# chenruduan/OAReactDiff

Hardware: AMD Instinct MI355X
Metric: denoising_steps_per_sec (higher is better)
Workload: dtype f32; 1 GPU; EGNNDynamics.forward (LEFTNet H=196 R=96 L=6), B=64 reactions/GPU x 3 objects x 23 atoms, complete graph per reaction (N=4416, E=300288), T=1000 sampler step shape; batch_per_gpu=64, atoms_per_object=23, parallelism=replica x1 (no collective), launch=eager

## Files before the change

### oareactdiff_amd/_capi.py

```python
from __future__ import annotations

import ctypes as C
import os

from .build import LIB

OARD_MAX_OBJECTS = 8
ABI_VERSION = 2040
OARD_OK, OARD_EINVAL, OARD_ENOTCOMPLETE, OARD_EHIP, OARD_ENOMEM = 0, -1, -2, -3, -4
ERRORS = {OARD_EINVAL: "invalid argument / unsupported configuration", OARD_ENOTCOMPLETE: "topology is not complete-per-sample",
          OARD_EHIP: "HIP runtime error", OARD_ENOMEM: "workspace too small"}

PREC_GCL_BF16X3, PREC_EQUI_BF16X3, PREC_TRAIN_BF16X3 = 1, 2, 4
TAP_S, TAP_VEC, TAP_EDGE, TAP_POS_FRAME, TAP_DPOS, TAP_HOUT, TAP_LABELS, TAP_NE1 = 1, 2, 3, 4, 5, 6, 7, 8

EXPORTS = ["oard_version", "oard_supported", "oard_param_count", "oard_packed_bytes", "oard_pack_weights",
           "oard_topology_create", "oard_topology_destroy", "oard_topology_num_nodes", "oard_topology_num_edges",
           "oard_topology_num_inner_edges", "oard_topology_num_samples", "oard_topology_check_edge_index",
           "oard_workspace_bytes", "oard_forward", "oard_active_inner_edges", "oard_debug_lin3u_table", "oard_sampler_step", "oard_sampler_step_dev", "oard_tap", "oard_debug_stop_after", "oard_debug_option", "oard_timing_enable", "oard_timing_reset",
           "oard_timing_get",
           "oard_topology_create_parts", "oard_topology_export", "oard_tape_bytes", "oard_tape_entry", "oard_forward_train",
           "oard_packed_bwd_bytes", "oard_pack_weights_bwd", "oard_gcl_backward_dx", "oard_edge_node_sums",
           "oard_equi_backward_dx", "oard_scalarize_backward", "oard_equi_msg_backward", "oard_lin3u_forward", "oard_lin3u_backward", "oard_wgrad_scratch_bytes", "oard_wgrad",
           "oard_train_scratch_bytes", "oard_train_scratch_poison", "oard_train_scratch_entry", "oard_train_tail_backward",
# ... 114 lines not shown
    L.oard_library_stream.argtypes = [ci, pvp]; L.oard_library_stream.restype = ci
    L.oard_graph_create.argtypes = [cfgp, vp, vp, i64, vp, i64, pvp]; L.oard_graph_create.restype = ci
    L.oard_graph_destroy.argtypes = [vp]; L.oard_graph_destroy.restype = None
    L.oard_graph_num_nodes.argtypes = [vp]; L.oard_graph_num_nodes.restype = i64
    L.oard_graph_num_edges.argtypes = [vp]; L.oard_graph_num_edges.restype = i64
    L.oard_graph_object_rows.argtypes = [vp, ci]; L.oard_graph_object_rows.restype = i64
    L.oard_graph_is_complete.argtypes = [vp]; L.oard_graph_is_complete.restype = ci
    L.oard_graph_workspace_bytes.argtypes = [cfgp, vp]; L.oard_graph_workspace_bytes.restype = sz
    L.oard_graph_forward.argtypes = [cfgp, vp, pvp, sz, pvp, vp, ci, vp, pvp, vp, sz, vp, vp]; L.oard_graph_forward.restype = ci
    L.oard_debug_stop_after.argtypes = [C.c_int]; L.oard_debug_stop_after.restype = C.c_int
    L.oard_debug_option.argtypes = [C.c_char_p, C.c_int]; L.oard_debug_option.restype = C.c_int
    L.oard_timing_enable.argtypes = [C.c_int]; L.oard_timing_enable.restype = C.c_int
    L.oard_timing_reset.argtypes = []; L.oard_timing_reset.restype = C.c_int
    L.oard_timing_get.argtypes = [C.c_char_p, C.POINTER(C.c_double), C.POINTER(i64)]; L.oard_timing_get.restype = C.c_int
    for env, opt in (("OARD_GCL_VARIANT", b"gcl_variant"), ("OARD_EQUI_VARIANT", b"equi_variant"),
                     ("OARD_NODE_VARIANT", b"node_variant"), ("OARD_GCL_SKIP", b"gcl_skip"), ("OARD_EQUI_SKIP", b"equi_skip"), ("OARD_EQUI_L0_SKIP", b"equi_l0_skip"), ("OARD_GCL_MSUM", b"gcl_msum"), ("OARD_GCL_PERSIST", b"gcl_persist"), ("OARD_GCL_GRID", b"gcl_grid"), ("OARD_PARTS", b"parts"), ("OARD_SEQUENTIAL", b"sequential"), ("OARD_POISON", b"poison"), ("OARD_AUTO_SMALL", b"auto_small"), ("OARD_AUTO_TINY", b"auto_tiny"), ("OARD_NPB", b"npb"),
                     ("OARD_WGRAD_WGS", b"wgrad_wgs"), ("OARD_WGRAD_LDS", b"wgrad_lds"), ("OARD_WGRAD_T16", b"wgrad_t16"), ("OARD_WGRAD_QUEUE", b"wgrad_queue"), ("OARD_GATE_FOLD", b"gate_fold"), ("OARD_WGRAD_SHAPES", b"wgrad_shapes"), ("OARD_TRAIN_DUAL", b"train_dual"), ("OARD_SMALL_SPLIT", b"small_split"),
                     ("OARD_SKIP_FAMILIES", b"skip_families")):
        if os.environ.get(env) not in (None, ""):
            check(L.oard_debug_option(opt, int(os.environ[env])), f"oard_debug_option({opt.decode()})")
    _lib = L
    return L


def timing_get(family: str):
    ms, n = C.c_double(0.0), C.c_int64(0)
    check(lib().oard_timing_get(family.encode(), C.byref(ms), C.byref(n)), "oard_timing_get")
    return ms.value, n.value
```

### oareactdiff_amd/csrc/oard_hip.hip

```cpp
#include <algorithm>
#include <cmath>
#include <cstdio>
#include <cstring>
#include <map>
#include <string>
#include <vector>
#include <mutex>
#include <chrono>
#include <utility>

#include "oard_kernels.h"
#include "oard_edge_v1.h"
#include "oard_edge_p.h"
#include "oard_wgrad_t16.h"
#include "oard_edge_b3.h"
#ifdef OARD_EXPERIMENTS
#include "oard_edge_fp.h"
#endif
#include "oard_node_v1.h"
#include "oard_edge_small.h"
#include "oard_edge_bwd.h"
#include "oard_node_bwd.h"
#include "oard_rows.h"
#include "oard_inst.h"
// ... 33 lines not shown
        }
        recs.clear();
    }
} g_timing;
int g_stop_after = 0;
int g_gcl_variant = 2;
int g_equi_variant = 2;
int g_sequential = 0;
int g_auto_tiny = 8;
int g_auto_small = 4;
int g_npb = 0;
int g_poison = 0;
int g_equi_l0_skip = 1;
int g_gcl_msum = 1;
int g_gcl_msum_taken = 0;
int g_equi_l0_taken = 0;
int g_parts = 0;
int g_small_split = 128;
int g_wgrad_shapes = 3;
int g_wgrad_t16 = 256;
int g_wgrad_lds = 256;
int g_wgrad_wgs = 512;
int g_gcl_persist = 1;
int g_gcl_grid = 0;
int g_equi_skip = 1;
int g_gcl_skip = 1;
int g_node_variant = 1;
int g_skip_families = 0;

struct ScopedLaunch {
// ... 517 lines not shown
    } else if constexpr (kV0) {
        LAUNCH(F_INIT, (k_neighbor<D>), gN, 256, st, tp, wb, po, (const float*)zemb, (const float*)nb, (const float*)ew, s_at(0), s1);
        LAUNCH(F_INIT, (k_s2v_agg<D>), gN, 256, st, tp, (const float*)s1, (const float*)ew, (const float*)geo, ne1);
    } else return OARD_EINVAL;
    if (A > 0) LAUNCH2(F_INIT, (k_scalarize<D>), gA, (gA * topo->conc <= 2048 ? D::HT : 1), 256, st, tp, wb, po, (const float*)ne1, (const float*)geo, ew);
    HIP_TRY(hipMemsetAsync(vec, 0, (size_t)N * 3 * D::HP * sizeof(float), st));
    if (stop_after == 1) return OARD_OK;

    float* vec2 = (float*)(ws + w.vec2);
    float* vcur = vec;
    float* vnext = vec2;
    const bool msum = !train && g_gcl_msum && E > 0 && gcl_variant == 2 && node_variant == 1 && equi_variant != 0 && tp.npb > 4 &&
                      (tp.CI == 0 || gcl_v1_throughput(c->precision, gcl_variant, topo->conc, tp.CI)) &&
                      (tp.CX == 0 || gcl_v1_throughput(c->precision, gcl_variant, topo->conc, tp.CX));
    g_gcl_msum_taken = msum;
    for (int l = 0; l < c->num_layers; ++l) {
        const LayerOff lo = po.layer[l];
        const bool nv1 = node_variant == 1 && equi_variant != 0;
        const unsigned gN16 = (unsigned)cdiv(N, tp.npb);
        float* ew_in = ew_at(l);
        float* ew_out = ew_at(l + 1);
        if (train) vnext = (float*)(tape + to.vec_in[l + 1]);

        if (nv1) LAUNCH(F_NODE, (k_node_pre_v1<D, NW>), gN16, NW * 64, st, tp, wb, po, lo, (const float*)s_at(l), (const float*)pp0, xhb, P, Q);
        else if constexpr (kV0) LAUNCH(F_NODE, (k_node_pre<D>), gN, 256, st, tp, wb, po, lo, (const float*)s, (const float*)pp0, xhb, P, Q);
        else return OARD_EINVAL;
        if (E > 0) {
            if (gcl_variant == 0) {
                if constexpr (kV0) LAUNCH(F_GCL_EDGE, (k_gcl_edge<D>), gE, 256, st, tp, wb, lo, (const float*)P, (const float*)Q, ew_in, mbuf);
                else return OARD_EINVAL;
// ... 23 lines not shown
                       s, vcur, v2buf, scal, vdot);
            } else return OARD_EINVAL;
        } else {
            const bool l0_skip = l == 0 && !train && g_equi_l0_skip && A > 0 && nv1 && !rows &&
                                 equi_v1_shape(c->precision, equi_variant, topo->conc, A, (const float*)(ws + w.d1s)) == 2;
            if (l == 0) g_equi_l0_taken = l0_skip;
            if (A > 0) {
                int rc = launch_equi_v1<D>(c->precision, equi_variant, topo->conc, tp, wb, lo, wb + lo.equi_stream, wb + lo.dp0b, ew_out, rbuf, vmsg,
                                           train ? (float*)(tape + to.zd1[l]) : nullptr, train ? (float*)(tape + to.cd[l]) : nullptr, st,
                                           (float*)(ws + w.d1s), al, l0_skip);
                if (rc != OARD_OK) return rc;
            }
#define EQUI_NODE_V1(D_, ROWS_, XC_) LAUNCH(F_NODE, (k_equi_node_v1<D_, NW, ROWS_, XC_>), gN16, NW * 64, st, tp, wb, lo, (const float*)vmsg, \
                       (const float*)xq, (const float*)geo, (const float*)x1, (const float*)s_mid_at(l), s_at(l + 1), (const float*)vcur, vnext, \
                       train ? (float*)(tape + to.s_a[l]) : nullptr, train ? (float*)(tape + to.vec_a[l]) : nullptr, al)
            if (nv1 && rows) {
                if (lo.xcross) EQUI_NODE_V1(D, true, true); else EQUI_NODE_V1(D, true, false);
            } else if (nv1 && l0_skip) {
                if (lo.xcross) EQUI_NODE_V1(Layer0<D>, false, true); else EQUI_NODE_V1(Layer0<D>, false, false);
            } else if (nv1) {
                if (lo.xcross) EQUI_NODE_V1(D, false, true); else EQUI_NODE_V1(D, false, false);
            } else if constexpr (kV0) {
                LAUNCH(F_NODE, (k_equi_agg_v1<D>), gN, 256, st, tp, wb, lo, (const float*)vmsg, (const float*)xq,
                       (const float*)geo, (const float*)x1, s, (const float*)vcur, vnext, v2buf, scal, vdot);
            } else return OARD_EINVAL;
            std::swap(vcur, vnext);
        }
        if constexpr (kV0) {
            if (!nv1) LAUNCH(F_NODE, (k_equi_upd<D>), gN, 256, st, tp, wb, lo, (const float*)scal, (const float*)vdot,
                             (const float*)v2buf, s, vcur);
        }
        if (stop_after == 100 + 10 * l + 2) { topo->vec_final = (size_t)((char*)vcur - ws); return OARD_OK; }
// ... 1535 lines not shown
    return OARD_OK;
}

int oard_debug_stop_after(int code) { g_stop_after = code; return OARD_OK; }
int oard_debug_option(const char* name, int value) {
    if (!name) return OARD_EINVAL;
    if (!kV0 && value == 0 && (strcmp(name, "gcl_variant") == 0 || strcmp(name, "equi_variant") == 0 || strcmp(name, "node_variant") == 0))
        return OARD_EINVAL;
    if (strcmp(name, "gcl_variant") == 0) { g_gcl_variant = value; return OARD_OK; }
    if (strcmp(name, "equi_variant") == 0) { g_equi_variant = value; return OARD_OK; }
    if (strcmp(name, "node_variant") == 0) { g_node_variant = value; return OARD_OK; }
    if (strcmp(name, "experiments") == 0) return kV0 ? OARD_OK : OARD_EINVAL;
    if (strcmp(name, "gcl_skip") == 0) { g_gcl_skip = value; return OARD_OK; }
    if (strcmp(name, "equi_skip") == 0) { g_equi_skip = value; return OARD_OK; }
    if (strcmp(name, "equi_l0_skip") == 0) { g_equi_l0_skip = value; return OARD_OK; }
    if (strcmp(name, "gcl_msum") == 0) { g_gcl_msum = value; return OARD_OK; }
    if (strcmp(name, "gcl_msum_taken") == 0) return g_gcl_msum_taken ? OARD_OK : OARD_EINVAL;
    if (strcmp(name, "equi_l0_taken") == 0) return g_equi_l0_taken ? OARD_OK : OARD_EINVAL;
    if (strcmp(name, "gcl_persist") == 0) { g_gcl_persist = value; return OARD_OK; }
    if (strcmp(name, "gcl_grid") == 0) { g_gcl_grid = value; return OARD_OK; }
    if (strcmp(name, "skip_families") == 0) { g_skip_families = value; return OARD_OK; }
    if (strcmp(name, "parts") == 0) { g_parts = value; return OARD_OK; }
    if (strcmp(name, "sequential") == 0) { g_sequential = value; return OARD_OK; }
    if (strcmp(name, "poison") == 0) { g_poison = value; return OARD_OK; }
    if (strcmp(name, "auto_small") == 0) { g_auto_small = value; return OARD_OK; }
    if (strcmp(name, "auto_tiny") == 0) { g_auto_tiny = value; return OARD_OK; }
    if (strcmp(name, "npb") == 0) { g_npb = value; return OARD_OK; }
    if (strcmp(name, "wgrad_wgs") == 0) { g_wgrad_wgs = value; return OARD_OK; }
    if (strcmp(name, "wgrad_t16") == 0) { g_wgrad_t16 = value; return OARD_OK; }
    if (strcmp(name, "wgrad_queue") == 0) { g_wgrad_queue = value; return OARD_OK; }
// ... 49 lines not shown
```

### oareactdiff_amd/csrc/oard_inst.h

```cpp
#pragma once
#if !defined(OARD_EXPERIMENTS) && !defined(OARD_SINGLE_TU)

#define OARD_UNPAREN(...) __VA_ARGS__
#ifdef OARD_INST_DEFINE
#define OARD_INST(K, ARGS) template __global__ void OARD_UNPAREN K ARGS;
#else
#define OARD_INST(K, ARGS) extern template __global__ void OARD_UNPAREN K ARGS;
#endif
#ifndef OARD_DIMS_LIST
#define OARD_DIMS_LIST X(196, 96) X(32, 8) X(32, 32)
#endif
#define OARD_BOOL4(M, D) M(D, true, true) M(D, false, true) M(D, true, false) M(D, false, false)

#define OARD_NW(h) (((h) + 15) / 16 <= 16 ? ((h) + 15) / 16 : 8)
#define OARD_A_GCL (TopoDev, const float*, const float*, const float*, const float*, const float*, long long, long long, const float*, float*, float*, GclTape)

#if !defined(OARD_INST_DEFINE) || defined(OARD_INST_UNIT_GCL_P)
#define OARD_I_GCL_P(D, S1, S3) OARD_INST((k_gcl_edge_p<OARD_UNPAREN D, S1, S3, false>), OARD_A_GCL) OARD_INST((k_gcl_edge_p<OARD_UNPAREN D, S1, S3, true>), OARD_A_GCL) \
    OARD_INST((k_gcl_edge_p<OARD_UNPAREN D, S1, S3, false, true>), OARD_A_GCL)
#define X(h, r) OARD_BOOL4(OARD_I_GCL_P, (Dims<h, r>))
OARD_DIMS_LIST
#undef X
#endif

// ... 24 lines not shown
    OARD_INST((k_equi_edge_v1<Dims<h, r>, 4, false>), OARD_A_EQUI) \
    OARD_INST((k_equi_node_v1<Dims<h, r>, OARD_NW(h), false, false>), OARD_A_EQUI_NODE) OARD_INST((k_equi_node_v1<Dims<h, r>, OARD_NW(h), false, true>), OARD_A_EQUI_NODE) \
    OARD_INST((k_equi_node_v1<Dims<h, r>, OARD_NW(h), true, false>), OARD_A_EQUI_NODE) OARD_INST((k_equi_node_v1<Dims<h, r>, OARD_NW(h), true, true>), OARD_A_EQUI_NODE) \
    OARD_INST((k_equi_node_v1<Layer0<Dims<h, r> >, OARD_NW(h), false, false>), OARD_A_EQUI_NODE) OARD_INST((k_equi_node_v1<Layer0<Dims<h, r> >, OARD_NW(h), false, true>), OARD_A_EQUI_NODE) \
    OARD_INST((k_gcl_edge_bwd<Dims<h, r>, 8, 2, true>), (TopoDev, const float*, long long, long long, GclBwdArgs)) \
    OARD_INST((k_gcl_edge_bwd<Dims<h, r>, 8, 2, false>), (TopoDev, const float*, long long, long long, GclBwdArgs)) \
    OARD_INST((k_equi_edge_bwd<Dims<h, r>, 8>), (TopoDev, const float*, const float*, const float*, float*, float*))
OARD_DIMS_LIST
#undef X
#endif

#if !defined(OARD_INST_DEFINE) || defined(OARD_INST_UNIT_NODE)
#define OARD_A_GCL_NODE (TopoDev, const float*, LayerOff, const float*, const float*, float*, float*, float*)
#define OARD_A_OUT (TopoDev, const float*, PackOff, const float*, const float*, float*, float*, int*)
#define OARD_A_SCAL_BWD (TopoDev, const float*, const float*, int, const float*, const float*, float*, float*)
#define OARD_A_MSG_BWD (TopoDev, const float*, Strided3, Strided3, const float*, Strided3, const float*, int, Strided3, float*, float*, float*, float*, int, int, int)
#define X(h, r) \
    OARD_INST((k_gcl_node_v1<Dims<h, r>, OARD_NW(h), false>), OARD_A_GCL_NODE) OARD_INST((k_gcl_node_v1<Dims<h, r>, OARD_NW(h), true>), OARD_A_GCL_NODE) \
    OARD_INST((k_gcl_node_v1<Dims<h, r>, OARD_NW(h), false, true>), OARD_A_GCL_NODE) \
    OARD_INST((k_out_v1<Dims<h, r>, OARD_NW(h)>), OARD_A_OUT) \
    OARD_INST((k_scalarize_bwd<Dims<h, r>, 2, false>), OARD_A_SCAL_BWD) OARD_INST((k_scalarize_bwd<Dims<h, r>, 2, true>), OARD_A_SCAL_BWD) \
    OARD_INST((k_equi_msg_bwd<Dims<h, r> >), OARD_A_MSG_BWD)
OARD_DIMS_LIST
#undef X
OARD_INST((k_lin3u_bwd_fused<4>), (const float*, const float*, const float*, long long, float*, float*))
#define OARD_I_ROWS(KB, EPI) OARD_INST((k_rows_dense<KB, EPI, 8>), (RowsDense)) OARD_INST((k_rows_dense_long<KB, EPI, 8, 4>), (RowsDense))
OARD_I_ROWS(13, 0) OARD_I_ROWS(13, 2) OARD_I_ROWS(13, 3) OARD_I_ROWS(7, 3) OARD_I_ROWS(6, 0) OARD_I_ROWS(6, 1) OARD_I_ROWS(4, 1) OARD_I_ROWS(4, 3)
OARD_INST((k_rows_dense<26, 1, 8>), (RowsDense)) OARD_INST((k_rows_dense<26, 3, 8>), (RowsDense))
OARD_INST((k_rows_dense2<13, 1, 8, 13>), (RowsDense2)) OARD_INST((k_rows_dense2<13, 2, 8, 13>), (RowsDense2))
OARD_INST((k_rows_dense2<26, 1, 8, 13>), (RowsDense2)) OARD_INST((k_rows_dense2<39, 2, 8, 13>), (RowsDense2))
#endif

#if !defined(OARD_INST_DEFINE) || defined(OARD_INST_UNIT_WGRAD)
#define OARD_A_WG (const float*, int, int, const float*, int, int, long long, long long, long long, int, int, float*, float*, float*)
OARD_INST((k_wgrad_t16<4, 7, false>), (WgtArgs)) OARD_INST((k_wgrad_t16<4, 7, true>), (WgtArgs)) OARD_INST((k_wgrad_t16<5, 3, false>), (WgtArgs))
OARD_INST((k_wgrad_t16<5, 5, true>), (WgtArgs)) OARD_INST((k_wgrad_t16<5, 7, true>), (WgtArgs)) OARD_INST((k_wgrad_t16<6, 5, false>), (WgtArgs))
OARD_INST((k_wgrad_t16<6, 7, false>), (WgtArgs))
// ... 7 lines not shown
```

### oareactdiff_amd/csrc/oard_node_v1.h

```cpp
#pragma once
#include "oard_kernels.h"

OARD_DEV f4 lds_blk(const float* v, int b, int lane) { return *reinterpret_cast<const f4*>(v + b * 256 + lane * 4); }
OARD_DEV void lds_st(float* v, int t, int lane, f4 x) { *reinterpret_cast<f4*>(v + t * 256 + lane * 4) = x; }

#ifndef OARD_NODE_PF
#define OARD_NODE_PF 13
#endif
template <int KB>
OARD_DEV f4 dense_tile_lds(const float* __restrict__ wp, int t, const float* in, int lane, f4 init) {
    const float* base = wp + ((size_t)t * KB * 64 + lane) * 4;
    f4 c0 = init, c1 = f4zero();
    constexpr int G = OARD_NODE_PF;
#pragma unroll
    for (int b0 = 0; b0 < KB; b0 += G) {
        f4 a[G];
#pragma unroll
        for (int i = 0; i < G; ++i)
            if (b0 + i < KB) a[i] = ld_f4(base + (size_t)(b0 + i) * 256);
        __builtin_amdgcn_sched_barrier(0);
#pragma unroll
        for (int i = 0; i < G; ++i)
            if (b0 + i < KB) {
                const f4 x = lds_blk(in, b0 + i, lane);
// ... 431 lines not shown
#pragma unroll
    for (int j = 0; j < 8; ++j) h2[j] = b2[j];
#pragma unroll 4
    for (int k = 0; k < 48; ++k) {
        const f4 wa = *reinterpret_cast<const f4*>(l3s + 12 * k), wc = *reinterpret_cast<const f4*>(l3s + 12 * k + 4);
        const float h = silu1(x * l3s[12 * k + 8] + l3s[12 * k + 9]);
        h2[0] += h * wa.x; h2[1] += h * wa.y; h2[2] += h * wa.z; h2[3] += h * wa.w;
        h2[4] += h * wc.x; h2[5] += h * wc.y; h2[6] += h * wc.z; h2[7] += h * wc.w;
    }
    float o = p[592];
#pragma unroll
    for (int j = 0; j < 8; ++j) o += silu1(h2[j]) * w4[j];
    return o;
}

template <class D> struct Layer0 : D {};
template <class D> struct is_layer0 { static constexpr bool value = false; };
template <class D> struct is_layer0<Layer0<D> > { static constexpr bool value = true; };
template <class D, int WAVES, bool ROWS = false, bool XC = false>
__global__ __launch_bounds__(WAVES * 64) void k_equi_node_v1(TopoDev tp, const float* __restrict__ wb, LayerOff lo,
                                                             const float* __restrict__ qbuf, const float* __restrict__ xq,
                                                             const float* __restrict__ geo, const float* __restrict__ x1,
                                                             const float* s, float* s_out, const float* __restrict__ vec_in,
                                                             float* __restrict__ vec_out,
                                                             float* __restrict__ sa_out, float* __restrict__ va_out ,
                                                             ActList al ) {
    constexpr bool L0 = is_layer0<D>::value;
    static_assert(!(L0 && ROWS), "the layer-0 form exists for the large-batch gather only");
    constexpr int HT = D::HT;
    constexpr int TPW = (HT + WAVES - 1) / WAVES;
    __shared__ __attribute__((aligned(16))) float sm[6 * HT * 256 + 48 * 12 + L3T_FLOATS];
    float* l3s = sm + 6 * HT * 256;
    float* l3t = l3s + 48 * 12;
#ifdef OARD_NO_L3T
    const bool l3t_ok = false;
#else
    const bool l3t_ok = tp.npb > 4 && (wb + lo.l3t)[2 * (L3T_N + 1)] > 0.5f;
#endif
    if (l3t_ok)
        for (int i = threadIdx.x; i < 2 * (L3T_N + 1) / 4; i += WAVES * 64)
            reinterpret_cast<f4*>(l3t)[i] = ld_f4(wb + lo.l3t + 4 * i);
    if (l3t_ok && threadIdx.x < 2) l3t[2 * (L3T_N + 1) - 2 + threadIdx.x] = (wb + lo.l3t)[2 * (L3T_N + 1) - 2 + threadIdx.x];
#ifdef OARD_TIMELINE
    const bool tl_on_ = blockIdx.x == gridDim.x / 2 && (threadIdx.x & 63) == 0; int tl_n_ = 0;
#endif
    TL(1);
    lin3u_stage(wb + lo.l3u, l3s, threadIdx.x, WAVES * 64);
    float* vx = sm;
    float* in = sm + 3 * HT * 256;
    float* hx = sm + 5 * HT * 256;
    const NodeBlk nb = node_blk(tp.N, tp.npb);
    const int n = nb.n;
    const bool listed = al.pre != nullptr && (long long)__builtin_amdgcn_readfirstlane(*al.n) != tp.A;
    const int a0 = listed ? al.pre[tp.act_ptr[n]] : tp.act_ptr[n];
    const int cnt = nb.valid ? (listed ? al.pre[tp.act_ptr[n + 1]] : tp.act_ptr[n + 1]) - a0 : 0;
    const int mx = wave_max(cnt);
    auto row_of = [&](int k) -> int { return listed ? al.rows[k] : k; };
// ... 16 lines not shown
                     zn2 = ld_blk(xq, nn, 3 * D::HP, 2 * HT + t, nb.lane);
            for (int k = 0; k < mx2; k += rl.L) {
                const int kk = k + rl.slot;
                const int ke = min(b0 + min(kk, max(cnt2 - 1, 0)), a_hi);
                const size_t a = cnt2 > 0 ? (size_t)row_of(ke) : 0;
                const int m = cnt2 > 0 ? src_of(ke) : 0;
                const float* gp = geo + a * GEO_STRIDE;
                const float gx = gp[2], gy = gp[3], gz = gp[4];
                const float cx = XC ? gp[5] : 0.f, cy = XC ? gp[6] : 0.f, cz = XC ? gp[7] : 0.f;
                const f4 q0 = ld_blk(qbuf, a, 3 * D::HP, t, nb.lane), q1 = ld_blk(qbuf, a, 3 * D::HP, HT + t, nb.lane),
                         q2 = ld_blk(qbuf, a, 3 * D::HP, 2 * HT + t, nb.lane);
                const f4 y0 = ld_blk(xq, m, 3 * D::HP, t, nb.lane), y1 = ld_blk(xq, m, 3 * D::HP, HT + t, nb.lane),
                         y2 = ld_blk(xq, m, 3 * D::HP, 2 * HT + t, nb.lane);
                const f4 w0 = ld_blk(vec_in, (size_t)m * 3 + 0, D::HP, t, nb.lane), w1 = ld_blk(vec_in, (size_t)m * 3 + 1, D::HP, t, nb.lane),
                         w2 = ld_blk(vec_in, (size_t)m * 3 + 2, D::HP, t, nb.lane);
                if (kk < cnt2) {
                    const f4 xm = (y0 + zn0) * q0;
                    dx += xm;
                    const f4 a2 = (y1 + zn1) * q1 * inv_sqrt3;
                    const f4 a3 = (y2 + zn2) * q2;
                    v0 += (XC ? w0 * a2 + a3 * gx + xm * cx : w0 * a2 + a3 * gx) * inv_sqrt_h;
                    v1 += (XC ? w1 * a2 + a3 * gy + xm * cy : w1 * a2 + a3 * gy) * inv_sqrt_h;
                    v2 += (XC ? w2 * a2 + a3 * gz + xm * cz : w2 * a2 + a3 * gz) * inv_sqrt_h;
                }
            }
            dx = rows_total4(dx, rl, nb.lane); v0 = rows_total4(v0, rl, nb.lane);
            v1 = rows_total4(v1, rl, nb.lane); v2 = rows_total4(v2, rl, nb.lane);
        }
        int mnext[2], rnext[2];
        auto entry = [&](int kk, int& m, int& r) {
            const int ke = min(a0 + min(kk, max(cnt - 1, 0)), a_hi);
            m = cnt > 0 ? src_of(ke) : 0;
            r = cnt > 0 ? row_of(ke) : 0;
        };
#pragma unroll
        for (int i = 0; i < 2; ++i) entry(i, mnext[i], rnext[i]);
        float zero1 = 0.f;
        if (L0) asm volatile("" : "+v"(zero1));
        const f4 zero4 = {zero1, zero1, zero1, zero1};
// ... 9 lines not shown
                const size_t a = (size_t)rc[i];
                const int m = mc[i];
                const float* g = geo + a * GEO_STRIDE;
                gx[i] = g[2]; gy[i] = g[3]; gz[i] = g[4];
                cx[i] = XC ? g[5] : 0.f; cy[i] = XC ? g[6] : 0.f; cz[i] = XC ? g[7] : 0.f;
                q0[i] = ld_blk(qbuf, a, 3 * D::HP, t, nb.lane); q1[i] = L0 ? zero4 : ld_blk(qbuf, a, 3 * D::HP, HT + t, nb.lane);
                q2[i] = ld_blk(qbuf, a, 3 * D::HP, 2 * HT + t, nb.lane);
                y0[i] = ld_blk(xq, m, 3 * D::HP, t, nb.lane); y1[i] = L0 ? zero4 : ld_blk(xq, m, 3 * D::HP, HT + t, nb.lane);
                y2[i] = ld_blk(xq, m, 3 * D::HP, 2 * HT + t, nb.lane);
                w0[i] = L0 ? zero4 : ld_blk(vec_in, (size_t)m * 3 + 0, D::HP, t, nb.lane);
                w1[i] = L0 ? zero4 : ld_blk(vec_in, (size_t)m * 3 + 1, D::HP, t, nb.lane);
                w2[i] = L0 ? zero4 : ld_blk(vec_in, (size_t)m * 3 + 2, D::HP, t, nb.lane);
            }
#pragma unroll
            for (int i = 0; i < 2; ++i)
                if (k + i < cnt) {
                    const f4 xm = (y0[i] + xn0) * q0[i];
                    dx += xm;
                    const f4 a2 = (y1[i] + xn1) * q1[i] * inv_sqrt3;
                    const f4 a3 = (y2[i] + xn2) * q2[i];
                    v0 += (XC ? w0[i] * a2 + a3 * gx[i] + xm * cx[i] : w0[i] * a2 + a3 * gx[i]) * inv_sqrt_h;
                    v1 += (XC ? w1[i] * a2 + a3 * gy[i] + xm * cy[i] : w1[i] * a2 + a3 * gy[i]) * inv_sqrt_h;
                    v2 += (XC ? w2[i] * a2 + a3 * gz[i] + xm * cz[i] : w2[i] * a2 + a3 * gz[i]) * inv_sqrt_h;
                }
        }
        const f4 sa = (ld_blk(s, n, D::HP, t, nb.lane) + dx) * inv_sqrt2;
        v0 += ld_blk(vec_in, (size_t)n * 3 + 0, D::HP, t, nb.lane);
        v1 += ld_blk(vec_in, (size_t)n * 3 + 1, D::HP, t, nb.lane);
        v2 += ld_blk(vec_in, (size_t)n * 3 + 2, D::HP, t, nb.lane);
        lds_st(in, t, nb.lane, sa);
        lds_st(vx + 0 * HT * 256, t, nb.lane, v0);
        lds_st(vx + 1 * HT * 256, t, nb.lane, v1);
        lds_st(vx + 2 * HT * 256, t, nb.lane, v2);
        if (sa_out != nullptr && nb.valid) {
            st_blk(sa_out, n, D::HP, t, nb.lane, sa);
            st_blk(va_out, (size_t)n * 3 + 0, D::HP, t, nb.lane, v0);
            st_blk(va_out, (size_t)n * 3 + 1, D::HP, t, nb.lane, v1);
            st_blk(va_out, (size_t)n * 3 + 2, D::HP, t, nb.lane, v2);
        }
    }
    TL(2);
    __syncthreads();
    TL(3);

    const float fx = x1[n * 3], fy = x1[n * 3 + 1], fz = x1[n * 3 + 2];
    const float* l3 = wb + lo.l3u;
    f4 v2k[TPW][3], vdk[TPW];
#pragma unroll
    for (int i = 0; i < TPW; ++i) {
        const int t = nb.wave + i * WAVES;
        if (t < HT) {
            TileJob job[2] = {tile_job<HT>(wb + lo.vp, t, vx), tile_job<HT>(wb + lo.vp, HT + t, vx)};
            f4 acc[6];
#pragma unroll
            for (int k = 0; k < 6; ++k) acc[k] = f4zero();
            dense_seq_xyz<HT, 2, HT * 256, (ROWS ? 5 : OARD_NODE_SEQ_G), ROWS>(job, nb.lane, acc);
            const f4 v1[3] = {acc[0], acc[1], acc[2]}, v2[3] = {acc[3], acc[4], acc[5]};
#pragma unroll
            for (int x = 0; x < 3; ++x) v2k[i][x] = v2[x];
            const f4 sc = v1[0] * fx + v1[1] * fy + v1[2] * fz;
            vdk[i] = (v1[0] * v2[0] + v1[1] * v2[1] + v1[2] * v2[2]) * inv_sqrt_h;
            f4 sca;
            const int f0 = 16 * t + 4 * nb.g;
            if (tp.npb <= 4) {
                float* blk = in + (HT + t) * 256;
                lds_st(in, HT + t, nb.lane, sc);
                __builtin_amdgcn_wave_barrier();
                const int f = nb.lane >> 2, c = nb.lane & 3;
                float* cell = blk + (16 * (f >> 2) + c) * 4 + (f & 3);
                const float y = (c < tp.npb && 16 * t + f < D::H) ? lin3u1(l3s, l3, *cell) : 0.f;
                *cell = y;
            } else {
                const bool in_tab = fabsf(sc.x) < L3T_X && fabsf(sc.y) < L3T_X && fabsf(sc.z) < L3T_X && fabsf(sc.w) < L3T_X;
                if (l3t_ok && !__any(!in_tab))
                    sca = (f4){lin3u_table_eval(l3t, sc.x), lin3u_table_eval(l3t, sc.y), lin3u_table_eval(l3t, sc.z), lin3u_table_eval(l3t, sc.w)};
                else
                    sca = lin3u4(l3s, l3, sc);
                sca.x = f0 + 0 < D::H ? sca.x : 0.f; sca.y = f0 + 1 < D::H ? sca.y : 0.f;
                sca.z = f0 + 2 < D::H ? sca.z : 0.f; sca.w = f0 + 3 < D::H ? sca.w : 0.f;
                lds_st(in, HT + t, nb.lane, sca);
            }
        }
    }
    TL(4);
    __syncthreads();
    TL(5);

    {
        TileJob job[TPW];
        f4 acc[TPW];
#pragma unroll
        for (int i = 0; i < TPW; ++i) { job[i] = tile_job<2 * HT>(wb + lo.xv0, min(nb.wave + i * WAVES, HT - 1), in); acc[i] = f4zero(); }
        dense_seq<2 * HT, TPW>(job, nb.lane, acc);
#pragma unroll
        for (int i = 0; i < TPW; ++i)
            if (nb.wave + i * WAVES < HT) lds_st(hx, nb.wave + i * WAVES, nb.lane, silu4(acc[i]));
    }
    TL(6);
    __syncthreads();
    TL(7);

    {
        TileJob job[3 * TPW];
        f4 acc[3 * TPW];
#pragma unroll
        for (int i = 0; i < TPW; ++i) {
            const int t = min(nb.wave + i * WAVES, HT - 1);
#pragma unroll
            for (int k = 0; k < 3; ++k) { job[3 * i + k] = tile_job<HT>(wb + lo.xv2, k * HT + t, hx); acc[3 * i + k] = f4zero(); }
        }
        dense_seq<HT, 3 * TPW>(job, nb.lane, acc);
#pragma unroll
        for (int i = 0; i < TPW; ++i) {
            const int t = nb.wave + i * WAVES;
            if (t < HT && nb.valid) {
                const f4 a = acc[3 * i], b = acc[3 * i + 1], c = acc[3 * i + 2];
                st_blk(s_out, n, D::HP, t, nb.lane, lds_blk(in, t, nb.lane) + (a + b + vdk[i]) * inv_sqrt2);
#pragma unroll
                for (int x = 0; x < 3; ++x)
                    st_blk(vec_out, (size_t)n * 3 + x, D::HP, t, nb.lane,
                           lds_blk(vx + x * HT * 256, t, nb.lane) + c * v2k[i][x]);
            }
        }
    }
    TL(0);
    TL_END();
}

template <class D, int WAVES>
__global__ __launch_bounds__(WAVES * 64) void k_neighbor_v1(TopoDev tp, const float* __restrict__ wb, PackOff po,
                                                            const float* __restrict__ zemb, const float* __restrict__ nbe,
                                                            const float* __restrict__ ew, float* __restrict__ s,
                                                            float* __restrict__ s1) {
    constexpr int HT = D::HT, TPW = (HT + WAVES - 1) / WAVES;
    __shared__ __attribute__((aligned(16))) float sm[2 * HT * 256];
    float* sv = sm;
    float* yv = sm + HT * 256;
    const NodeBlk nb = node_blk(tp.N, tp.npb);
    const int n = nb.n, smp = tp.node_sample[n], s0 = tp.sample_ptr[smp];
    const int ns = nb.valid ? tp.sample_ptr[smp + 1] - s0 : 0;
    const int mx = wave_max(ns);
// ... 210 lines not shown
```

Baseline: 3698 reaction-steps/s.

## Split equivariant node kernel into per-feature gather and dense update kernels

Adds an inference-only path that breaks the fused equivariant node kernel in two. A wave-per-64-features gather kernel accumulates edge messages directly from global memory into s and a vector buffer. A separate block-tiled update kernel then reloads those into LDS and runs the dense projections. The gather is meant to get better parallelism and latency hiding than the LDS-heavy fused kernel, at the cost of an extra kernel launch and a global round trip for the intermediate s/vec. The shared math is factored into helpers, and message accumulation now uses explicit FMAs with contraction disabled.

```diff
diff --git a/oareactdiff_amd/_capi.py b/oareactdiff_amd/_capi.py
--- a/oareactdiff_amd/_capi.py
+++ b/oareactdiff_amd/_capi.py
@@ -152,7 +152,7 @@
     L.oard_timing_reset.argtypes = []; L.oard_timing_reset.restype = C.c_int
     L.oard_timing_get.argtypes = [C.c_char_p, C.POINTER(C.c_double), C.POINTER(i64)]; L.oard_timing_get.restype = C.c_int
     for env, opt in (("OARD_GCL_VARIANT", b"gcl_variant"), ("OARD_EQUI_VARIANT", b"equi_variant"),
-                     ("OARD_NODE_VARIANT", b"node_variant"), ("OARD_GCL_SKIP", b"gcl_skip"), ("OARD_EQUI_SKIP", b"equi_skip"), ("OARD_EQUI_L0_SKIP", b"equi_l0_skip"), ("OARD_GCL_MSUM", b"gcl_msum"), ("OARD_GCL_PERSIST", b"gcl_persist"), ("OARD_GCL_GRID", b"gcl_grid"), ("OARD_PARTS", b"parts"), ("OARD_SEQUENTIAL", b"sequential"), ("OARD_POISON", b"poison"), ("OARD_AUTO_SMALL", b"auto_small"), ("OARD_AUTO_TINY", b"auto_tiny"), ("OARD_NPB", b"npb"),
+                     ("OARD_NODE_VARIANT", b"node_variant"), ("OARD_GCL_SKIP", b"gcl_skip"), ("OARD_EQUI_SKIP", b"equi_skip"), ("OARD_EQUI_L0_SKIP", b"equi_l0_skip"), ("OARD_EQUI_SPLIT", b"equi_split"), ("OARD_GCL_MSUM", b"gcl_msum"), ("OARD_GCL_PERSIST", b"gcl_persist"), ("OARD_GCL_GRID", b"gcl_grid"), ("OARD_PARTS", b"parts"), ("OARD_SEQUENTIAL", b"sequential"), ("OARD_POISON", b"poison"), ("OARD_AUTO_SMALL", b"auto_small"), ("OARD_AUTO_TINY", b"auto_tiny"), ("OARD_NPB", b"npb"),
                      ("OARD_WGRAD_WGS", b"wgrad_wgs"), ("OARD_WGRAD_LDS", b"wgrad_lds"), ("OARD_WGRAD_T16", b"wgrad_t16"), ("OARD_WGRAD_QUEUE", b"wgrad_queue"), ("OARD_GATE_FOLD", b"gate_fold"), ("OARD_WGRAD_SHAPES", b"wgrad_shapes"), ("OARD_TRAIN_DUAL", b"train_dual"), ("OARD_SMALL_SPLIT", b"small_split"),
                      ("OARD_SKIP_FAMILIES", b"skip_families")):
         if os.environ.get(env) not in (None, ""):
diff --git a/oareactdiff_amd/csrc/oard_hip.hip b/oareactdiff_amd/csrc/oard_hip.hip
--- a/oareactdiff_amd/csrc/oard_hip.hip
+++ b/oareactdiff_amd/csrc/oard_hip.hip
@@ -71,6 +71,8 @@
 int g_equi_l0_skip = 1;
 int g_gcl_msum = 1;
 int g_gcl_msum_taken = 0;
+int g_equi_split = 1;
+int g_equi_split_taken = 0;
 int g_equi_l0_taken = 0;
 int g_parts = 0;
 int g_small_split = 128;
@@ -618,6 +620,8 @@
                       (tp.CI == 0 || gcl_v1_throughput(c->precision, gcl_variant, topo->conc, tp.CI)) &&
                       (tp.CX == 0 || gcl_v1_throughput(c->precision, gcl_variant, topo->conc, tp.CX));
     g_gcl_msum_taken = msum;
+    const bool equi_split = !train && g_equi_split && A > 0 && node_variant == 1 && equi_variant != 0 && tp.npb > 4;
+    g_equi_split_taken = equi_split;
     for (int l = 0; l < c->num_layers; ++l) {
         const LayerOff lo = po.layer[l];
         const bool nv1 = node_variant == 1 && equi_variant != 0;
@@ -671,8 +675,14 @@
 #define EQUI_NODE_V1(D_, ROWS_, XC_) LAUNCH(F_NODE, (k_equi_node_v1<D_, NW, ROWS_, XC_>), gN16, NW * 64, st, tp, wb, lo, (const float*)vmsg, \
                        (const float*)xq, (const float*)geo, (const float*)x1, (const float*)s_mid_at(l), s_at(l + 1), (const float*)vcur, vnext, \
                        train ? (float*)(tape + to.s_a[l]) : nullptr, train ? (float*)(tape + to.vec_a[l]) : nullptr, al)
+#define EQUI_GATHER_V1(D_, XC_) LAUNCH(F_NODE, (k_equi_gather_v1<D_, XC_>), (unsigned)cdiv(N * ((D::HP + 63) / 64), 4), 256, st, tp, (const float*)vmsg, \
+                       (const float*)xq, (const float*)geo, s, (const float*)vcur, vnext, al)
             if (nv1 && rows) {
                 if (lo.xcross) EQUI_NODE_V1(D, true, true); else EQUI_NODE_V1(D, true, false);
+            } else if (nv1 && equi_split) {
+                if (l0_skip) { if (lo.xcross) EQUI_GATHER_V1(Layer0<D>, true); else EQUI_GATHER_V1(Layer0<D>, false); }
+                else { if (lo.xcross) EQUI_GATHER_V1(D, true); else EQUI_GATHER_V1(D, false); }
+                LAUNCH(F_NODE, (k_equi_update_v1<D, NW>), gN16, NW * 64, st, tp, wb, lo, (const float*)x1, s, vnext);
             } else if (nv1 && l0_skip) {
                 if (lo.xcross) EQUI_NODE_V1(Layer0<D>, false, true); else EQUI_NODE_V1(Layer0<D>, false, false);
             } else if (nv1) {
@@ -2238,6 +2248,8 @@
     if (strcmp(name, "gcl_skip") == 0) { g_gcl_skip = value; return OARD_OK; }
     if (strcmp(name, "equi_skip") == 0) { g_equi_skip = value; return OARD_OK; }
     if (strcmp(name, "equi_l0_skip") == 0) { g_equi_l0_skip = value; return OARD_OK; }
+    if (strcmp(name, "equi_split") == 0) { g_equi_split = value; return OARD_OK; }
+    if (strcmp(name, "equi_split_taken") == 0) return g_equi_split_taken ? OARD_OK : OARD_EINVAL;
     if (strcmp(name, "gcl_msum") == 0) { g_gcl_msum = value; return OARD_OK; }
     if (strcmp(name, "gcl_msum_taken") == 0) return g_gcl_msum_taken ? OARD_OK : OARD_EINVAL;
     if (strcmp(name, "equi_l0_taken") == 0) return g_equi_l0_taken ? OARD_OK : OARD_EINVAL;
diff --git a/oareactdiff_amd/csrc/oard_inst.h b/oareactdiff_amd/csrc/oard_inst.h
--- a/oareactdiff_amd/csrc/oard_inst.h
+++ b/oareactdiff_amd/csrc/oard_inst.h
@@ -62,13 +62,17 @@
 #define OARD_A_GCL_NODE (TopoDev, const float*, LayerOff, const float*, const float*, float*, float*, float*)
 #define OARD_A_OUT (TopoDev, const float*, PackOff, const float*, const float*, float*, float*, int*)
 #define OARD_A_SCAL_BWD (TopoDev, const float*, const float*, int, const float*, const float*, float*, float*)
+#define OARD_A_EQUI_GATHER (TopoDev, const float*, const float*, const float*, float*, const float*, float*, ActList)
 #define OARD_A_MSG_BWD (TopoDev, const float*, Strided3, Strided3, const float*, Strided3, const float*, int, Strided3, float*, float*, float*, float*, int, int, int)
 #define X(h, r) \
     OARD_INST((k_gcl_node_v1<Dims<h, r>, OARD_NW(h), false>), OARD_A_GCL_NODE) OARD_INST((k_gcl_node_v1<Dims<h, r>, OARD_NW(h), true>), OARD_A_GCL_NODE) \
     OARD_INST((k_gcl_node_v1<Dims<h, r>, OARD_NW(h), false, true>), OARD_A_GCL_NODE) \
     OARD_INST((k_out_v1<Dims<h, r>, OARD_NW(h)>), OARD_A_OUT) \
     OARD_INST((k_scalarize_bwd<Dims<h, r>, 2, false>), OARD_A_SCAL_BWD) OARD_INST((k_scalarize_bwd<Dims<h, r>, 2, true>), OARD_A_SCAL_BWD) \
-    OARD_INST((k_equi_msg_bwd<Dims<h, r> >), OARD_A_MSG_BWD)
+    OARD_INST((k_equi_msg_bwd<Dims<h, r> >), OARD_A_MSG_BWD) \
+    OARD_INST((k_equi_gather_v1<Dims<h, r>, false>), OARD_A_EQUI_GATHER) OARD_INST((k_equi_gather_v1<Dims<h, r>, true>), OARD_A_EQUI_GATHER) \
+    OARD_INST((k_equi_gather_v1<Layer0<Dims<h, r> >, false>), OARD_A_EQUI_GATHER) OARD_INST((k_equi_gather_v1<Layer0<Dims<h, r> >, true>), OARD_A_EQUI_GATHER) \
+    OARD_INST((k_equi_update_v1<Dims<h, r>, OARD_NW(h)>), (TopoDev, const float*, LayerOff, const float*, float*, float*))
 OARD_DIMS_LIST
 #undef X
 OARD_INST((k_lin3u_bwd_fused<4>), (const float*, const float*, const float*, long long, float*, float*))
diff --git a/oareactdiff_amd/csrc/oard_node_v1.h b/oareactdiff_amd/csrc/oard_node_v1.h
--- a/oareactdiff_amd/csrc/oard_node_v1.h
+++ b/oareactdiff_amd/csrc/oard_node_v1.h
@@ -469,6 +469,130 @@
     return o;
 }
 
+template <class T> OARD_DEV T fma_t(T a, T b, T c) { return __builtin_elementwise_fma(a, b, c); }
+template <bool XC, class T>
+OARD_DEV void equi_msg_acc(T& dx, T& v0, T& v1, T& v2, T y0, T y1, T y2, T xn0, T xn1, T xn2, T q0, T q1, T q2, T w0, T w1, T w2, float gx,
+                           float gy, float gz, float cx, float cy, float cz, float inv_sqrt3, float inv_sqrt_h) {
+#pragma clang fp contract(off)
+    const T s0 = y0 + xn0;
+    const T xm = s0 * q0;
+    dx = fma_t(s0, q0, dx);
+    const T a2 = (y1 + xn1) * q1 * inv_sqrt3;
+    const T a3 = (y2 + xn2) * q2;
+    T u0 = fma_t(w0, a2, a3 * gx), u1 = fma_t(w1, a2, a3 * gy), u2 = fma_t(w2, a2, a3 * gz);
+    if (XC) { u0 = fma_t(xm, (T)cx, u0); u1 = fma_t(xm, (T)cy, u1); u2 = fma_t(xm, (T)cz, u2); }
+    v0 = fma_t(u0, (T)inv_sqrt_h, v0);
+    v1 = fma_t(u1, (T)inv_sqrt_h, v1);
+    v2 = fma_t(u2, (T)inv_sqrt_h, v2);
+}
+#ifdef OARD_TIMELINE
+#define OARD_TL_PARAMS , const bool tl_on_, int& tl_n_
+#define OARD_TL_ARGS , tl_on_, tl_n_
+#else
+#define OARD_TL_PARAMS
+#define OARD_TL_ARGS
+#endif
+template <int WAVES>
+OARD_DEV bool equi_stage_l3t(const TopoDev& tp, const float* wb, const LayerOff& lo, float* l3t) {
+#ifdef OARD_NO_L3T
+    const bool l3t_ok = false;
+#else
+    const bool l3t_ok = tp.npb > 4 && (wb + lo.l3t)[2 * (L3T_N + 1)] > 0.5f;
+#endif
+    if (l3t_ok)
+        for (int i = threadIdx.x; i < 2 * (L3T_N + 1) / 4; i += WAVES * 64)
+            reinterpret_cast<f4*>(l3t)[i] = ld_f4(wb + lo.l3t + 4 * i);
+    if (l3t_ok && threadIdx.x < 2) l3t[2 * (L3T_N + 1) - 2 + threadIdx.x] = (wb + lo.l3t)[2 * (L3T_N + 1) - 2 + threadIdx.x];
+    return l3t_ok;
+}
+template <class D, int WAVES, bool ROWS>
+OARD_DEV void equi_update_stages(const int npb, const float* w_vp, const float* w_xv0, const float* w_xv2, const float* l3, const float* x1, float* s_out,
+                                 float* vec_out, float* vx, float* in, float* hx, const float* l3s, const float* l3t, const bool l3t_ok,
+                                 const NodeBlk& nb, const float inv_sqrt2, const float inv_sqrt_h OARD_TL_PARAMS) {
+    constexpr int HT = D::HT;
+    constexpr int TPW = (HT + WAVES - 1) / WAVES;
+    const int n = nb.n;
+    const float fx = x1[n * 3], fy = x1[n * 3 + 1], fz = x1[n * 3 + 2];
+    f4 v2k[TPW][3], vdk[TPW];
+#pragma unroll
+    for (int i = 0; i < TPW; ++i) {
+        const int t = nb.wave + i * WAVES;
+        if (t < HT) {
+            TileJob job[2] = {tile_job<HT>(w_vp, t, vx), tile_job<HT>(w_vp, HT + t, vx)};
+            f4 acc[6];
+#pragma unroll
+            for (int k = 0; k < 6; ++k) acc[k] = f4zero();
+            dense_seq_xyz<HT, 2, HT * 256, (ROWS ? 5 : OARD_NODE_SEQ_G), ROWS>(job, nb.lane, acc);
+            const f4 v1[3] = {acc[0], acc[1], acc[2]}, v2[3] = {acc[3], acc[4], acc[5]};
+#pragma unroll
+            for (int x = 0; x < 3; ++x) v2k[i][x] = v2[x];
+            const f4 sc = v1[0] * fx + v1[1] * fy + v1[2] * fz;
+            vdk[i] = (v1[0] * v2[0] + v1[1] * v2[1] + v1[2] * v2[2]) * inv_sqrt_h;
+            f4 sca;
+            const int f0 = 16 * t + 4 * nb.g;
+            if (npb <= 4) {
+                float* blk = in + (HT + t) * 256;
+                lds_st(in, HT + t, nb.lane, sc);
+                __builtin_amdgcn_wave_barrier();
+                const int f = nb.lane >> 2, c = nb.lane & 3;
+                float* cell = blk + (16 * (f >> 2) + c) * 4 + (f & 3);
+                const float y = (c < npb && 16 * t + f < D::H) ? lin3u1(l3s, l3, *cell) : 0.f;
+                *cell = y;
+            } else {
+                const bool in_tab = fabsf(sc.x) < L3T_X && fabsf(sc.y) < L3T_X && fabsf(sc.z) < L3T_X && fabsf(sc.w) < L3T_X;
+                if (l3t_ok && !__any(!in_tab))
+                    sca = (f4){lin3u_table_eval(l3t, sc.x), lin3u_table_eval(l3t, sc.y), lin3u_table_eval(l3t, sc.z), lin3u_table_eval(l3t, sc.w)};
+                else
+                    sca = lin3u4(l3s, l3, sc);
+                sca.x = f0 + 0 < D::H ? sca.x : 0.f; sca.y = f0 + 1 < D::H ? sca.y : 0.f;
+                sca.z = f0 + 2 < D::H ? sca.z : 0.f; sca.w = f0 + 3 < D::H ? sca.w : 0.f;
+                lds_st(in, HT + t, nb.lane, sca);
+            }
+        }
+    }
+    TL(4);
+    __syncthreads();
+    TL(5);
+
+    {
+        TileJob job[TPW];
+        f4 acc[TPW];
+#pragma unroll
+        for (int i = 0; i < TPW; ++i) { job[i] = tile_job<2 * HT>(w_xv0, min(nb.wave + i * WAVES, HT - 1), in); acc[i] = f4zero(); }
+        dense_seq<2 * HT, TPW>(job, nb.lane, acc);
+#pragma unroll
+        for (int i = 0; i < TPW; ++i)
+            if (nb.wave + i * WAVES < HT) lds_st(hx, nb.wave + i * WAVES, nb.lane, silu4(acc[i]));
+    }
+    TL(6);
+    __syncthreads();
+    TL(7);
+
+    {
+        TileJob job[3 * TPW];
+        f4 acc[3 * TPW];
+#pragma unroll
+        for (int i = 0; i < TPW; ++i) {
+            const int t = min(nb.wave + i * WAVES, HT - 1);
+#pragma unroll
+            for (int k = 0; k < 3; ++k) { job[3 * i + k] = tile_job<HT>(w_xv2, k * HT + t, hx); acc[3 * i + k] = f4zero(); }
+        }
+        dense_seq<HT, 3 * TPW>(job, nb.lane, acc);
+#pragma unroll
+        for (int i = 0; i < TPW; ++i) {
+            const int t = nb.wave + i * WAVES;
+            if (t < HT && nb.valid) {
+                const f4 a = acc[3 * i], b = acc[3 * i + 1], c = acc[3 * i + 2];
+                st_blk(s_out, n, D::HP, t, nb.lane, lds_blk(in, t, nb.lane) + (a + b + vdk[i]) * inv_sqrt2);
+#pragma unroll
+                for (int x = 0; x < 3; ++x)
+                    st_blk(vec_out, (size_t)n * 3 + x, D::HP, t, nb.lane,
+                           lds_blk(vx + x * HT * 256, t, nb.lane) + c * v2k[i][x]);
+            }
+        }
+    }
+}
+
 template <class D> struct Layer0 : D {};
 template <class D> struct is_layer0 { static constexpr bool value = false; };
 template <class D> struct is_layer0<Layer0<D> > { static constexpr bool value = true; };
@@ -487,15 +611,7 @@
     __shared__ __attribute__((aligned(16))) float sm[6 * HT * 256 + 48 * 12 + L3T_FLOATS];
     float* l3s = sm + 6 * HT * 256;
     float* l3t = l3s + 48 * 12;
-#ifdef OARD_NO_L3T
-    const bool l3t_ok = false;
-#else
-    const bool l3t_ok = tp.npb > 4 && (wb + lo.l3t)[2 * (L3T_N + 1)] > 0.5f;
-#endif
-    if (l3t_ok)
-        for (int i = threadIdx.x; i < 2 * (L3T_N + 1) / 4; i += WAVES * 64)
-            reinterpret_cast<f4*>(l3t)[i] = ld_f4(wb + lo.l3t + 4 * i);
-    if (l3t_ok && threadIdx.x < 2) l3t[2 * (L3T_N + 1) - 2 + threadIdx.x] = (wb + lo.l3t)[2 * (L3T_N + 1) - 2 + threadIdx.x];
+    const bool l3t_ok = equi_stage_l3t<WAVES>(tp, wb, lo, l3t);
 #ifdef OARD_TIMELINE
     const bool tl_on_ = blockIdx.x == gridDim.x / 2 && (threadIdx.x & 63) == 0; int tl_n_ = 0;
 #endif
@@ -542,15 +658,8 @@
                          y2 = ld_blk(xq, m, 3 * D::HP, 2 * HT + t, nb.lane);
                 const f4 w0 = ld_blk(vec_in, (size_t)m * 3 + 0, D::HP, t, nb.lane), w1 = ld_blk(vec_in, (size_t)m * 3 + 1, D::HP, t, nb.lane),
                          w2 = ld_blk(vec_in, (size_t)m * 3 + 2, D::HP, t, nb.lane);
-                if (kk < cnt2) {
-                    const f4 xm = (y0 + zn0) * q0;
-                    dx += xm;
-                    const f4 a2 = (y1 + zn1) * q1 * inv_sqrt3;
-                    const f4 a3 = (y2 + zn2) * q2;
-                    v0 += (XC ? w0 * a2 + a3 * gx + xm * cx : w0 * a2 + a3 * gx) * inv_sqrt_h;
-                    v1 += (XC ? w1 * a2 + a3 * gy + xm * cy : w1 * a2 + a3 * gy) * inv_sqrt_h;
-                    v2 += (XC ? w2 * a2 + a3 * gz + xm * cz : w2 * a2 + a3 * gz) * inv_sqrt_h;
-                }
+                if (kk < cnt2)
+                    equi_msg_acc<XC>(dx, v0, v1, v2, y0, y1, y2, zn0, zn1, zn2, q0, q1, q2, w0, w1, w2, gx, gy, gz, cx, cy, cz, inv_sqrt3, inv_sqrt_h);
             }
             dx = rows_total4(dx, rl, nb.lane); v0 = rows_total4(v0, rl, nb.lane);
             v1 = rows_total4(v1, rl, nb.lane); v2 = rows_total4(v2, rl, nb.lane);
@@ -590,15 +699,9 @@
             }
 #pragma unroll
             for (int i = 0; i < 2; ++i)
-                if (k + i < cnt) {
-                    const f4 xm = (y0[i] + xn0) * q0[i];
-                    dx += xm;
-                    const f4 a2 = (y1[i] + xn1) * q1[i] * inv_sqrt3;
-                    const f4 a3 = (y2[i] + xn2) * q2[i];
-                    v0 += (XC ? w0[i] * a2 + a3 * gx[i] + xm * cx[i] : w0[i] * a2 + a3 * gx[i]) * inv_sqrt_h;
-                    v1 += (XC ? w1[i] * a2 + a3 * gy[i] + xm * cy[i] : w1[i] * a2 + a3 * gy[i]) * inv_sqrt_h;
-                    v2 += (XC ? w2[i] * a2 + a3 * gz[i] + xm * cz[i] : w2[i] * a2 + a3 * gz[i]) * inv_sqrt_h;
-                }
+                if (k + i < cnt)
+                    equi_msg_acc<XC>(dx, v0, v1, v2, y0[i], y1[i], y2[i], xn0, xn1, xn2, q0[i], q1[i], q2[i], w0[i], w1[i], w2[i], gx[i], gy[i], gz[i],
+                                     cx[i], cy[i], cz[i], inv_sqrt3, inv_sqrt_h);
         }
         const f4 sa = (ld_blk(s, n, D::HP, t, nb.lane) + dx) * inv_sqrt2;
         v0 += ld_blk(vec_in, (size_t)n * 3 + 0, D::HP, t, nb.lane);
@@ -619,88 +722,109 @@
     __syncthreads();
     TL(3);
 
-    const float fx = x1[n * 3], fy = x1[n * 3 + 1], fz = x1[n * 3 + 2];
-    const float* l3 = wb + lo.l3u;
-    f4 v2k[TPW][3], vdk[TPW];
-#pragma unroll
-    for (int i = 0; i < TPW; ++i) {
-        const int t = nb.wave + i * WAVES;
-        if (t < HT) {
-            TileJob job[2] = {tile_job<HT>(wb + lo.vp, t, vx), tile_job<HT>(wb + lo.vp, HT + t, vx)};
-            f4 acc[6];
-#pragma unroll
-            for (int k = 0; k < 6; ++k) acc[k] = f4zero();
-            dense_seq_xyz<HT, 2, HT * 256, (ROWS ? 5 : OARD_NODE_SEQ_G), ROWS>(job, nb.lane, acc);
-            const f4 v1[3] = {acc[0], acc[1], acc[2]}, v2[3] = {acc[3], acc[4], acc[5]};
-#pragma unroll
-            for (int x = 0; x < 3; ++x) v2k[i][x] = v2[x];
-            const f4 sc = v1[0] * fx + v1[1] * fy + v1[2] * fz;
-            vdk[i] = (v1[0] * v2[0] + v1[1] * v2[1] + v1[2] * v2[2]) * inv_sqrt_h;
-            f4 sca;
-            const int f0 = 16 * t + 4 * nb.g;
-            if (tp.npb <= 4) {
-                float* blk = in + (HT + t) * 256;
-                lds_st(in, HT + t, nb.lane, sc);
-                __builtin_amdgcn_wave_barrier();
-                const int f = nb.lane >> 2, c = nb.lane & 3;
-                float* cell = blk + (16 * (f >> 2) + c) * 4 + (f & 3);
-                const float y = (c < tp.npb && 16 * t + f < D::H) ? lin3u1(l3s, l3, *cell) : 0.f;
-                *cell = y;
-            } else {
-                const bool in_tab = fabsf(sc.x) < L3T_X && fabsf(sc.y) < L3T_X && fabsf(sc.z) < L3T_X && fabsf(sc.w) < L3T_X;
-                if (l3t_ok && !__any(!in_tab))
-                    sca = (f4){lin3u_table_eval(l3t, sc.x), lin3u_table_eval(l3t, sc.y), lin3u_table_eval(l3t, sc.z), lin3u_table_eval(l3t, sc.w)};
-                else
-                    sca = lin3u4(l3s, l3, sc);
-                sca.x = f0 + 0 < D::H ? sca.x : 0.f; sca.y = f0 + 1 < D::H ? sca.y : 0.f;
-                sca.z = f0 + 2 < D::H ? sca.z : 0.f; sca.w = f0 + 3 < D::H ? sca.w : 0.f;
-                lds_st(in, HT + t, nb.lane, sca);
-            }
-        }
-    }
-    TL(4);
-    __syncthreads();
-    TL(5);
-
-    {
-        TileJob job[TPW];
-        f4 acc[TPW];
-#pragma unroll
-        for (int i = 0; i < TPW; ++i) { job[i] = tile_job<2 * HT>(wb + lo.xv0, min(nb.wave + i * WAVES, HT - 1), in); acc[i] = f4zero(); }
-        dense_seq<2 * HT, TPW>(job, nb.lane, acc);
-#pragma unroll
-        for (int i = 0; i < TPW; ++i)
-            if (nb.wave + i * WAVES < HT) lds_st(hx, nb.wave + i * WAVES, nb.lane, silu4(acc[i]));
-    }
-    TL(6);
-    __syncthreads();
-    TL(7);
-
-    {
-        TileJob job[3 * TPW];
-        f4 acc[3 * TPW];
-#pragma unroll
-        for (int i = 0; i < TPW; ++i) {
-            const int t = min(nb.wave + i * WAVES, HT - 1);
-#pragma unroll
-            for (int k = 0; k < 3; ++k) { job[3 * i + k] = tile_job<HT>(wb + lo.xv2, k * HT + t, hx); acc[3 * i + k] = f4zero(); }
-        }
-        dense_seq<HT, 3 * TPW>(job, nb.lane, acc);
-#pragma unroll
-        for (int i = 0; i < TPW; ++i) {
-            const int t = nb.wave + i * WAVES;
-            if (t < HT && nb.valid) {
-                const f4 a = acc[3 * i], b = acc[3 * i + 1], c = acc[3 * i + 2];
-                st_blk(s_out, n, D::HP, t, nb.lane, lds_blk(in, t, nb.lane) + (a + b + vdk[i]) * inv_sqrt2);
-#pragma unroll
-                for (int x = 0; x < 3; ++x)
-                    st_blk(vec_out, (size_t)n * 3 + x, D::HP, t, nb.lane,
-                           lds_blk(vx + x * HT * 256, t, nb.lane) + c * v2k[i][x]);
-            }
-        }
-    }
+    equi_update_stages<D, WAVES, ROWS>(tp.npb, wb + lo.vp, wb + lo.xv0, wb + lo.xv2, wb + lo.l3u, x1, s_out, vec_out, vx, in, hx, l3s, l3t, l3t_ok, nb, inv_sqrt2, inv_sqrt_h OARD_TL_ARGS);
     TL(0);
     TL_END();
+}
+
+template <class D, bool XC>
+__global__ __launch_bounds__(256) void k_equi_gather_v1(TopoDev tp, const float* __restrict__ qbuf, const float* __restrict__ xq,
+                                                        const float* __restrict__ geo, float* s, const float* __restrict__ vec_in,
+                                                        float* __restrict__ va, ActList al) {
+    constexpr bool L0 = is_layer0<D>::value;
+    constexpr int HP = D::HP, CH = (HP + 63) / 64, EF = 4;
+    const int lane = threadIdx.x & 63;
+    const long long wv = (long long)blockIdx.x * 4 + __builtin_amdgcn_readfirstlane((int)(threadIdx.x >> 6));
+    if (wv >= (long long)tp.N * CH) return;
+    const int n = (int)(wv / CH), f = (int)(wv % CH) * 64 + lane;
+    const bool live = f < HP;
+    const int fc = live ? f : HP - 1;
+    const bool listed = al.pre != nullptr && (long long)*al.n != tp.A;
+    const int a0 = listed ? al.pre[tp.act_ptr[n]] : tp.act_ptr[n];
+    const int cnt = (listed ? al.pre[tp.act_ptr[n + 1]] : tp.act_ptr[n + 1]) - a0;
+    const int a_hi = (int)max(tp.A - 1, 0LL);
+    const float inv_sqrt2 = 0.70710678118654752f, inv_sqrt3 = 0.57735026918962576f, inv_sqrt_h = 1.0f / sqrtf((float)D::H);
+    const int* srcs = listed ? al.src : tp.act_src;
+    const int* rows = listed ? al.rows : tp.act_src;
+    auto entry = [&](int kk, int& m, int& r) {
+        const int ke = min(a0 + min(kk, max(cnt - 1, 0)), a_hi);
+        const int rr = rows[ke];
+        m = srcs[ke];
+        r = listed ? rr : ke;
+    };
+    const float* xn = xq + (size_t)n * (3 * HP) + fc;
+    const float xn0 = xn[0], xn1 = xn[HP], xn2 = xn[2 * HP];
+    float zero1 = 0.f;
+    if (L0) asm volatile("" : "+v"(zero1));
+    float dx = 0.f, v0 = 0.f, v1 = 0.f, v2 = 0.f;
+    int mnext[EF], rnext[EF];
+#pragma unroll
+    for (int i = 0; i < EF; ++i) entry(i, mnext[i], rnext[i]);
+    auto step = [&](const int k, const bool full) {
+        float q0[EF], q1[EF], q2[EF], y0[EF], y1[EF], y2[EF], w0[EF], w1[EF], w2[EF];
+        float gx[EF], gy[EF], gz[EF], cx[EF], cy[EF], cz[EF];
+        int mc[EF], rc[EF];
+#pragma unroll
+        for (int i = 0; i < EF; ++i) { mc[i] = mnext[i]; rc[i] = rnext[i]; }
+#pragma unroll
+        for (int i = 0; i < EF; ++i) entry(k + EF + i, mnext[i], rnext[i]);
+#pragma unroll
+        for (int i = 0; i < EF; ++i) {
+            const float* g = geo + (size_t)rc[i] * GEO_STRIDE;
+            gx[i] = g[2]; gy[i] = g[3]; gz[i] = g[4];
+            cx[i] = XC ? g[5] : 0.f; cy[i] = XC ? g[6] : 0.f; cz[i] = XC ? g[7] : 0.f;
+            const float* q = qbuf + (size_t)rc[i] * (3 * HP) + fc;
+            const float* y = xq + (size_t)mc[i] * (3 * HP) + fc;
+            const float* w = vec_in + (size_t)mc[i] * (3 * HP) + fc;
+            q0[i] = q[0]; q1[i] = L0 ? zero1 : q[HP]; q2[i] = q[2 * HP];
+            y0[i] = y[0]; y1[i] = L0 ? zero1 : y[HP]; y2[i] = y[2 * HP];
+            w0[i] = L0 ? zero1 : w[0]; w1[i] = L0 ? zero1 : w[HP]; w2[i] = L0 ? zero1 : w[2 * HP];
+        }
+#pragma unroll
+        for (int i = 0; i < EF; ++i)
+            if (full || k + i < cnt)
+                equi_msg_acc<XC>(dx, v0, v1, v2, y0[i], y1[i], y2[i], xn0, xn1, xn2, q0[i], q1[i], q2[i], w0[i], w1[i], w2[i], gx[i], gy[i], gz[i],
+                                 cx[i], cy[i], cz[i], inv_sqrt3, inv_sqrt_h);
+    };
+    int k = 0;
+    for (; k + EF <= cnt; k += EF) step(k, true);
+    if (k < cnt) step(k, false);
+    float* sp = s + (size_t)n * HP + fc;
+    const float* vi = vec_in + (size_t)n * (3 * HP) + fc;
+    const float sa = (*sp + dx) * inv_sqrt2;
+    v0 += vi[0]; v1 += vi[HP]; v2 += vi[2 * HP];
+    if (live) {
+        float* vo = va + (size_t)n * (3 * HP) + f;
+        *sp = sa;
+        vo[0] = v0; vo[HP] = v1; vo[2 * HP] = v2;
+    }
+}
+
+template <class D, int WAVES>
+__global__ __launch_bounds__(WAVES * 64) void k_equi_update_v1(TopoDev tp, const float* __restrict__ wb, LayerOff lo, const float* __restrict__ x1,
+                                                               float* s, float* vec) {
+    constexpr int HT = D::HT;
+    __shared__ __attribute__((aligned(16))) float sm[6 * HT * 256 + 48 * 12 + L3T_FLOATS];
+    float* l3s = sm + 6 * HT * 256;
+    float* l3t = l3s + 48 * 12;
+    const bool l3t_ok = equi_stage_l3t<WAVES>(tp, wb, lo, l3t);
+#ifdef OARD_TIMELINE
+    const bool tl_on_ = false; int tl_n_ = 0;
+#endif
+    lin3u_stage(wb + lo.l3u, l3s, threadIdx.x, WAVES * 64);
+    float* vx = sm;
+    float* in = sm + 3 * HT * 256;
+    float* hx = sm + 5 * HT * 256;
+    const NodeBlk nb = node_blk(tp.N, tp.npb);
+    const float inv_sqrt2 = 0.70710678118654752f, inv_sqrt_h = 1.0f / sqrtf((float)D::H);
+    for (int t = nb.wave; t < HT; t += WAVES) {
+        lds_st(in, t, nb.lane, ld_blk(s, nb.n, D::HP, t, nb.lane));
+#pragma unroll
+        for (int x = 0; x < 3; ++x) lds_st(vx + x * HT * 256, t, nb.lane, ld_blk(vec, (size_t)nb.n * 3 + x, D::HP, t, nb.lane));
+    }
+    __syncthreads();
+    equi_update_stages<D, WAVES, false>(tp.npb, wb + lo.vp, wb + lo.xv0, wb + lo.xv2, wb + lo.l3u, x1, s, vec, vx, in, hx, l3s, l3t, l3t_ok, nb,
+                                        inv_sqrt2, inv_sqrt_h OARD_TL_ARGS);
 }
 
 template <class D, int WAVES>
```

New measurement: 3731 reaction-steps/s (median of 6 runs). No clear change (+0.9%).
